# FluxML/Flux3D.jl

Hardware: AMD Instinct MI355X
Metric: chamfer_point_pairs_per_sec (higher is better)
Workload: dtype f32

## Files before the change

flux3d.jl_amd/csrc/chamfer.hip:

```cpp
#include <cmath>

#include "nn1_common.h"

using namespace fx3d;

#ifdef FX3D_PROBE
__device__ unsigned long long g_probe[4096 * 16];
#define FX3D_PROBE_MARK(k)                                                                   \
    do {                                                                                     \
        if (threadIdx.x == 0 && blockIdx.x < 4096) {                                         \
            g_probe[blockIdx.x * 16 + (k)] = __builtin_readcyclecounter();                   \
            if ((k) == 0) g_probe[blockIdx.x * 16 + 13] = wall_clock64();                    \
            if ((k) == 12) g_probe[blockIdx.x * 16 + 14] = wall_clock64();                   \
        }                                                                                    \
    } while (0)
__device__ unsigned long long g_probe2[256 * 16];
#define FX3D_PROBE_MARK2(k) do { if (threadIdx.x == 0 && blockIdx.x < 256) g_probe2[blockIdx.x * 16 + (k)] = __builtin_readcyclecounter(); } while (0)
__device__ unsigned long long g_probe3[16 * 16 * 8];
#define FX3D_PROBE_MARKW(k) do { if ((threadIdx.x & 63) == 0 && blockIdx.x < 16) g_probe3[(blockIdx.x * 16 + (threadIdx.x >> 6)) * 8 + (k)] = __builtin_readcyclecounter(); } while (0)
#else
#define FX3D_PROBE_MARK(k) do { } while (0)
#define FX3D_PROBE_MARK2(k) do { } while (0)
#define FX3D_PROBE_MARKW(k) do { } while (0)
#endif

namespace {

__device__ __forceinline__ void load4pts(const float *__restrict__ base, int p0, float (&px)[4],
                                         float (&py)[4], float (&pz)[4]) {
    const float4 *s4 = reinterpret_cast<const float4 *>(base + (size_t)p0 * 3);
    const float4 f0 = s4[0], f1 = s4[1], f2 = s4[2];
    px[0] = f0.x; py[0] = f0.y; pz[0] = f0.z;
    px[1] = f0.w; py[1] = f1.x; pz[1] = f1.y;
    px[2] = f1.z; py[2] = f1.w; pz[2] = f2.x;
    px[3] = f2.y; py[3] = f2.z; pz[3] = f2.w;
}

typedef _Float16 h8 __attribute__((ext_vector_type(8)));
typedef float f32x16 __attribute__((ext_vector_type(16)));
#ifndef FX3D_HFIFO
#define FX3D_HFIFO 5
#endif
constexpr int kHFifo = FX3D_HFIFO;
#ifndef FX3D_HRUNS_FROM
#define FX3D_HRUNS_FROM 16
#endif
constexpr int kHRunsFrom = FX3D_HRUNS_FROM;
constexpr int kScanU = 2;
#ifndef FX3D_HRUNCAP
#define FX3D_HRUNCAP 384
#endif
constexpr int kHRunCap = FX3D_HRUNCAP;
constexpr int kHItemCap = 64 * kHFifo > kHRunCap ? 64 * kHFifo : kHRunCap;
constexpr int kHFarCap = 64;
#ifndef FX3D_HBLKTRACK
#define FX3D_HBLKTRACK 1
#endif
constexpr bool kHBlkTrack = FX3D_HBLKTRACK != 0;
constexpr int kHIdBits = kHBlkTrack ? 7 : 6;
static_assert(kHChunkMax / (32 * kHLT) <= 64, "lane-tile ids live in the six (block ids: seven) low mantissa bits of the tracked keys");
constexpr float kKeyUp = kHBlkTrack ? 0x1.2p-16f : 0x1.2p-17f;
constexpr float kPadF16 = 65504.0f;
__device__ const unsigned short kHilbertCell[512] = {
    0, 1, 65, 64, 72, 73, 9, 8, 16, 24, 88, 80, 81, 89, 25, 17, 18, 26, 27, 19, 83, 91, 90, 82, 74, 10, 11, 75, 67, 3, 2, 66,
    130, 194, 195, 131, 139, 203, 202, 138, 146, 154, 155, 147, 211, 219, 218, 210, 209, 217, 153, 145, 144, 152, 216, 208, 200, 201, 137, 136, 128, 129, 193, 192,
    256, 257, 265, 264, 328, 329, 321, 320, 384, 448, 456, 392, 393, 457, 449, 385, 386, 450, 451, 387, 395, 459, 458, 394, 330, 322, 323, 331, 267, 259, 258, 266,
    274, 282, 283, 275, 339, 347, 346, 338, 402, 466, 467, 403, 411, 475, 474, 410, 409, 473, 465, 401, 400, 464, 472, 408, 344, 345, 337, 336, 272, 273, 281, 280,
    288, 296, 297, 289, 353, 361, 360, 352, 416, 480, 481, 417, 425, 489, 488, 424, 432, 496, 504, 440, 441, 505, 497, 433, 369, 368, 376, 377, 313, 312, 304, 305,
    306, 307, 315, 314, 378, 379, 371, 370, 434, 498, 506, 442, 443, 507, 499, 435, 427, 491, 490, 426, 418, 482, 483, 419, 355, 363, 362, 354, 290, 298, 299, 291,
    227, 235, 171, 163, 162, 170, 234, 226, 225, 224, 160, 161, 169, 168, 232, 233, 241, 240, 248, 249, 185, 184, 176, 177, 178, 242, 250, 186, 187, 251, 243, 179,
    115, 51, 59, 123, 122, 58, 50, 114, 113, 112, 120, 121, 57, 56, 48, 49, 41, 40, 104, 105, 97, 96, 32, 33, 34, 42, 106, 98, 99, 107, 43, 35,
    36, 44, 108, 100, 101, 109, 45, 37, 38, 39, 103, 102, 110, 111, 47, 46, 54, 55, 63, 62, 126, 127, 119, 118, 117, 53, 61, 125, 124, 60, 52, 116,
    180, 244, 252, 188, 189, 253, 245, 181, 182, 183, 191, 190, 254, 255, 247, 246, 238, 239, 175, 174, 166, 167, 231, 230, 229, 237, 173, 165, 164, 172, 236, 228,
    292, 300, 301, 293, 357, 365, 364, 356, 420, 484, 485, 421, 429, 493, 492, 428, 436, 500, 508, 444, 445, 509, 501, 437, 373, 372, 380, 381, 317, 316, 308, 309,
    310, 311, 319, 318, 382, 383, 375, 374, 438, 502, 510, 446, 447, 511, 503, 439, 431, 495, 494, 430, 422, 486, 487, 423, 359, 367, 366, 358, 294, 302, 303, 295,
    287, 286, 278, 279, 343, 342, 350, 351, 415, 479, 471, 407, 406, 470, 478, 414, 413, 477, 476, 412, 404, 468, 469, 405, 341, 349, 348, 340, 276, 284, 285, 277,
    269, 261, 260, 268, 332, 324, 325, 333, 397, 461, 460, 396, 388, 452, 453, 389, 390, 454, 462, 398, 399, 463, 455, 391, 327, 326, 334, 335, 271, 270, 262, 263,
    199, 198, 134, 135, 143, 142, 206, 207, 215, 223, 159, 151, 150, 158, 222, 214, 213, 221, 220, 212, 148, 156, 157, 149, 141, 205, 204, 140, 132, 196, 197, 133,
    69, 5, 4, 68, 76, 12, 13, 77, 85, 93, 92, 84, 20, 28, 29, 21, 22, 30, 94, 86, 87, 95, 31, 23, 15, 14, 78, 79, 71, 70, 6, 7,
};
constexpr size_t kHScratchBytes = (kHThreads / 64) * (32 * 8 + kHItemCap * 2 + 32 * 3 * 4) + 64 * 32;

__device__ __forceinline__ float vmin(float a, float b) {
    float r;
    asm("v_min_f32 %0, %1, %2" : "=v"(r) : "v"(a), "v"(b));
    return r;
}

__device__ __forceinline__ void split2h(float v, _Float16 &h, _Float16 &l) {
    h = (_Float16)v;
    l = (_Float16)(v - (float)h);
}

constexpr float kBetaC = 0x1.1p-18f;
constexpr float kBandB1 = 1.0f + 18.0f * kBetaC + 0x1p-20f;
constexpr float kBandA = 22.3f * kBetaC + 0x1p-19f;
__device__ __forceinline__ void make_pieces(float cx, float cy, float cz, h8 &p0, h8 &p1) {
    _Float16 hx, lx, hy, ly, hz, lz, n1, n2, n3;
    split2h(cx, hx, lx); split2h(cy, hy, ly); split2h(cz, hz, lz);
    const float n0 = ((cx * cx) + (cy * cy)) + (cz * cz);
    const float n = n0 + kBetaC * n0;
    n1 = (_Float16)n;
    const float r1 = n - (float)n1;
    n2 = (_Float16)r1;
    n3 = (_Float16)(r1 - (float)n2);
    const _Float16 z = (_Float16)0.0f;
    p0 = h8{hx, hx, lx, hy, hy, ly, hz, hz};
    p1 = h8{lz, n1, n2, n3, lx, ly, lz, z};
}

template <bool WANT_IDX, bool SPLITFUSE = false, bool PRUNE = false>
__global__ __launch_bounds__(kHThreads, 4) void nn1_f16_kernel(Nn1Params p) {
    extern __shared__ __attribute__((aligned(16))) float lds[];
    __shared__ __attribute__((aligned(16))) float red[4 * 4 * (kHThreads / 64) + 16];
    __shared__ int nfar[2];
    __shared__ unsigned short farlist[kHFarCap];
    constexpr int QB = (kHThreads / 64) * 32;

    const int L = blockIdx.x;
    const int per_cloud = p.tiles * p.nsplit;
    const bool by_xcd = 2 * p.B >= 8;
    const int slot = by_xcd ? L >> 3 : L;
    const int c = by_xcd ? (slot / per_cloud) * 8 + (L & 7) : slot / per_cloud;
    const int tile = (slot % per_cloud) / p.nsplit;
    const int split = (slot % per_cloud) % p.nsplit;
    if (c >= 2 * p.B) return;
    const int dir = c >= p.B ? 1 : 0;
    const int b = dir ? c - p.B : c;
    const int NQ = dir ? p.M : p.N;
    const int NC = dir ? p.N : p.M;
    if (tile >= (dir ? p.tiles_y : p.tiles_x)) return;
    if ((long long)split * p.chunk >= NC) return;
    const int ctail = (p.tail > 0 && p.nsplit == 1 && NC > p.chunk && NC - p.chunk <= p.tail) ? NC - p.chunk : 0;
    const int NCm = NC - ctail;
    const float *__restrict__ qb = (dir ? p.y : p.x) + (size_t)b * NQ * 3;
    const float *__restrict__ cb = (dir ? p.x : p.y) + (size_t)b * NC * 3;
    int32_t *idx_out = dir ? p.idx_y : p.idx_x;
    float *dmin_out = dir ? p.dmin_y : p.dmin_x;

    const int tid = threadIdx.x, lane = tid & 63;
    const int wv = __builtin_amdgcn_readfirstlane(tid >> 6);
    const int jq = lane & 31, hh = lane >> 5;
    const int CH = p.chunk;
    const int tpb = dir ? p.tpb_y : p.tpb;
    h8 *imgp = reinterpret_cast<h8 *>(lds);
    float4 *imgf = reinterpret_cast<float4 *>(lds);
    unsigned long long *wres = reinterpret_cast<unsigned long long *>(lds + 8 * (CH + 64));
    unsigned short *witems = reinterpret_cast<unsigned short *>(wres + (kHThreads / 64) * 32);
    float *wq = reinterpret_cast<float *>(witems + (kHThreads / 64) * kHItemCap);
    unsigned long long *qres = wres + wv * 32;
    unsigned short *items = witems + wv * kHItemCap;
    float *qtab = wq + wv * 96;
    const bool vec = (reinterpret_cast<uintptr_t>(cb) & 15) == 0;
    const bool one_shot = NCm <= CH;
    if (tid == 0) { nfar[0] = 0; nfar[1] = 0; }
    float qpre[3];
    {
        const int q0i = (tile * tpb) * QB + wv * 32 + jq;
        const int qc0 = q0i < NQ ? q0i : NQ - 1;
#pragma unroll
        for (int d = 0; d < 3; ++d) qpre[d] = qb[(size_t)qc0 * 3 + d];
    }
    if constexpr (PRUNE) {
        unsigned int *zc = reinterpret_cast<unsigned int *>(wres);
        for (int i = tid; i < 1040 + 16 * 256; i += kHThreads) zc[i] = 0u;
        int *gb = reinterpret_cast<int *>(wq + (kHThreads / 64) * 96) + 64 * 8;
        for (int i = tid; i < kHGroupsMax * 8; i += kHThreads) gb[i] = (i & 4) ? (int)0x80000000 : 0x7fffffff;
    }
    FX3D_PROBE_MARK(0);

    const bool own_chunk_only = p.nsplit > 1 && (long long)split * CH + (long long)p.nsplit * CH >= NCm;
    const int s_lo = own_chunk_only ? split * CH : 0;
    const int SN = own_chunk_only ? (NCm - s_lo < CH ? NCm - s_lo : CH) : NC;
    const float *__restrict__ sb = cb + (size_t)s_lo * 3;
    const bool parked = one_shot || own_chunk_only;
    float mu[3], cinf = 0.0f, varmax = 0.0f;
    float bxlo[3] = {0.f, 0.f, 0.f}, bxhi[3] = {0.f, 0.f, 0.f};
    bool allfin = true;
    {
        float mn[3] = {INFINITY, INFINITY, INFINITY}, mx[3] = {-INFINITY, -INFINITY, -INFINITY}, sm3[3] = {0.f, 0.f, 0.f};
        float sqt = 0.0f;
        const float pil[3] = {sb[0], sb[1], sb[2]};
        const int nsweep = (SN + kHThreads - 1) / kHThreads;
        for (int i0 = 0; i0 < nsweep; i0 += 4) {
            P3 v[4];
#pragma unroll
            for (int e = 0; e < 4; ++e) {
                const int pt = (i0 + e) * kHThreads + tid;
                v[e] = *reinterpret_cast<const P3 *>(sb + (size_t)(pt < SN ? pt : SN - 1) * 3);
            }
#pragma unroll
            for (int e = 0; e < 4; ++e) {
                const int pt = (i0 + e) * kHThreads + tid;
                mn[0] = fminf(mn[0], v[e].x); mx[0] = fmaxf(mx[0], v[e].x);
                mn[1] = fminf(mn[1], v[e].y); mx[1] = fmaxf(mx[1], v[e].y);
                mn[2] = fminf(mn[2], v[e].z); mx[2] = fmaxf(mx[2], v[e].z);
                if (pt < SN) {
                    sm3[0] = sm3[0] + v[e].x; sm3[1] = sm3[1] + v[e].y; sm3[2] = sm3[2] + v[e].z;
                    if (parked) imgf[((pt >> 5) * 2) * 32 + (pt & 31)] = float4{v[e].x, v[e].y, v[e].z, 0.0f};
                }
                if (((i0 + e) & 3) == (wv & 3) && pt < SN) {
                    sqt = __builtin_fmaf(v[e].x - pil[0], v[e].x - pil[0], sqt); sqt = __builtin_fmaf(v[e].y - pil[1], v[e].y - pil[1], sqt);
                    sqt = __builtin_fmaf(v[e].z - pil[2], v[e].z - pil[2], sqt);
                }
            }
        }
        FX3D_PROBE_MARK(5);
        {
            float4 lo4, hi4, st4;
            lo4.x = wave_min_l63(mn[0]); lo4.y = wave_min_l63(mn[1]); lo4.z = wave_min_l63(mn[2]); lo4.w = 0.0f;
            hi4.x = wave_max_l63(mx[0]); hi4.y = wave_max_l63(mx[1]); hi4.z = wave_max_l63(mx[2]); hi4.w = 0.0f;
            st4.x = wave_sum_l63(sm3[0]); st4.y = wave_sum_l63(sm3[1]); st4.z = wave_sum_l63(sm3[2]); st4.w = wave_sum_l63(sqt);
            if (lane == 63) {
                float4 *r4 = reinterpret_cast<float4 *>(red);
                r4[wv * 4] = lo4; r4[wv * 4 + 1] = hi4; r4[wv * 4 + 2] = st4;
            }
        }
        FX3D_PROBE_MARK(9);
        __syncthreads();
        FX3D_PROBE_MARK(10);
        static_assert(kHThreads / 64 == 16, "the cross-wave reduction below: one wave's row of 16 lanes, one lane per wave");
        if (wv == 0) {
            const float4 *r4 = reinterpret_cast<const float4 *>(red);
            const int w = lane & 15;
            float4 lo4 = r4[w * 4], hi4 = r4[w * 4 + 1], st4 = r4[w * 4 + 2];
#define NN1_ROW_MIN(v) v = fkey_inv(row_mm_key<false>(fkey(v)));
#define NN1_ROW_MAX(v) v = fkey_inv(row_mm_key<true>(fkey(v)));
#define NN1_ROW_SUM(v) v = v + dpp_mov<0xB1>(v); v = v + dpp_mov<0x4E>(v); v = v + dpp_mov<0x141>(v); v = v + dpp_mov<0x140>(v);
            NN1_ROW_MIN(lo4.x) NN1_ROW_MIN(lo4.y) NN1_ROW_MIN(lo4.z)
            NN1_ROW_MAX(hi4.x) NN1_ROW_MAX(hi4.y) NN1_ROW_MAX(hi4.z)
            NN1_ROW_SUM(st4.x) NN1_ROW_SUM(st4.y) NN1_ROW_SUM(st4.z) NN1_ROW_SUM(st4.w)
#undef NN1_ROW_MIN
#undef NN1_ROW_MAX
#undef NN1_ROW_SUM
            const float lo3[3] = {lo4.x, lo4.y, lo4.z}, hi3[3] = {hi4.x, hi4.y, hi4.z}, st3[3] = {st4.x, st4.y, st4.z};
            float m3[3], ci = 0.0f, vm = st4.w / fmaxf(0.25f * (float)SN, 1.0f);
            bool fin = true;
#pragma unroll
            for (int d = 0; d < 3; ++d) {
                const float lo = lo3[d], hi = hi3[d], st = st3[d];
                m3[d] = fminf(fmaxf(st / (float)SN, lo), hi);
                const float off = st / (float)SN - pil[d];
                vm = vm - off * off;
                ci = fmaxf(ci, fmaxf(hi - m3[d], m3[d] - lo));
                fin = fin && fabsf(st) < INFINITY;
            }
            if (lane == 0) {
                float4 *o4 = reinterpret_cast<float4 *>(red) + 4 * (kHThreads / 64);
                o4[0] = float4{m3[0], m3[1], m3[2], ci * 1.000001f};
                o4[1] = float4{vm, fin ? 1.0f : 0.0f, 0.0f, 0.0f};
                if (PRUNE) { o4[2] = float4{lo3[0], lo3[1], lo3[2], 0.0f}; o4[3] = float4{hi3[0], hi3[1], hi3[2], 0.0f}; }
            }
        }
        __syncthreads();
        {
            const float4 *o4 = reinterpret_cast<const float4 *>(red) + 4 * (kHThreads / 64);
            const float4 a = o4[0], b2 = o4[1];
            mu[0] = a.x; mu[1] = a.y; mu[2] = a.z; cinf = a.w;
            varmax = b2.x; allfin = b2.y != 0.0f;
            if (PRUNE) {
                const float4 l4 = o4[2], h4 = o4[3];
                bxlo[0] = l4.x; bxlo[1] = l4.y; bxlo[2] = l4.z; bxhi[0] = h4.x; bxhi[1] = h4.y; bxhi[2] = h4.z;
            }
        }
    }
    float rng = cinf;
    if (allfin && cinf < 1.0e16f && 3.0f * cinf * cinf > kRobustGate * varmax) {
        const float4 r = robust_range3<kHThreads, false>(sb, SN, parked, imgf, red, mu[0], mu[1], mu[2], cinf);
        mu[0] = r.x; mu[1] = r.y; mu[2] = r.z; rng = r.w;
    }
    const bool sane = allfin && cinf < 1.0e16f;
    float sc = 1.0f;
    if (sane && rng > 1.0e-30f) {
        int e;
        (void)frexpf(rng, &e);
        sc = ldexpf(1.0f, 7 - e);
    }
    auto uni = [](float v) { return __builtin_bit_cast(float, __builtin_amdgcn_readfirstlane(__builtin_bit_cast(int, v))); };
    mu[0] = uni(mu[0]); mu[1] = uni(mu[1]); mu[2] = uni(mu[2]); sc = uni(sc); rng = uni(rng); cinf = uni(cinf);
    const bool has_far = sane && rng < cinf;
    int fslot = 0;
    auto pieces = [&](float x, float y, float z, int pt, h8 &p0, h8 &p1) {
        const float sx = (x - mu[0]) * sc, sy = (y - mu[1]) * sc, sz = (z - mu[2]) * sc;
        if (!has_far) { make_pieces(sx, sy, sz, p0, p1); return; }
        const bool far = !(fmaxf(fmaxf(fabsf(sx), fabsf(sy)), fabsf(sz)) < 128.0f);
        make_pieces(far ? 0.f : sx, far ? 0.f : sy, far ? 0.f : sz, p0, p1);
        if (far) {
            p1[7] = (_Float16)kPadF16;
            const int f = atomicAdd(&nfar[fslot], 1);
            if (f < kHFarCap) farlist[f] = (unsigned short)pt;
        }
    };

    [[maybe_unused]] float4 *cs = nullptr, *qsw = nullptr;
    [[maybe_unused]] bool sorted_c = false;
    [[maybe_unused]] int qwlen = 0;
    [[maybe_unused]] float4 *boxes = nullptr;
    if constexpr (PRUNE) {
        cs = p.pscr + (size_t)blockIdx.x * p.pscr_stride;
        qsw = cs + kHChunkMax;
        boxes = reinterpret_cast<float4 *>(wq + (kHThreads / 64) * 96);
        unsigned int *ccnt = reinterpret_cast<unsigned int *>(wres);
        unsigned int *qtot = ccnt + 520;
        unsigned int *qwh = qtot + 520;
        const bool last_t = tile == (dir ? p.tiles_y : p.tiles_x) - 1;
        const int qw0 = tile * tpb * QB;
        const int qw1 = last_t || qw0 + tpb * QB > NQ ? NQ : qw0 + tpb * QB;
        qwlen = qw1 - qw0;
        const int cnt = NCm;
        const bool do_sort = sane && cnt >= 512;
        const bool sorted_q = do_sort && NQ <= 4 * kHThreads;
        P3 qv[4];
        if (sorted_q) {
#pragma unroll
            for (int e = 0; e < 4; ++e) {
                const int qp = 256 * wv + 64 * e + lane;
                qv[e] = *reinterpret_cast<const P3 *>(qb + (size_t)(qp < NQ ? qp : NQ - 1) * 3);
            }
        }
        FX3D_PROBE_MARK2(0);
        int *gbox = reinterpret_cast<int *>(boxes + 64 * 2);
        auto group_box = [&](int wrow, float x, float y, float z) {
            int *g = gbox + (wrow >> 5) * 8;
            atomicMin(g + 0, fkey((x - mu[0]) * sc)); atomicMin(g + 1, fkey((y - mu[1]) * sc)); atomicMin(g + 2, fkey((z - mu[2]) * sc));
            atomicMax(g + 4, fkey((x - mu[0]) * sc)); atomicMax(g + 5, fkey((y - mu[1]) * sc)); atomicMax(g + 6, fkey((z - mu[2]) * sc));
        };
        if (do_sort) {
            float4 cv[4];
#pragma unroll
            for (int e = 0; e < 4; ++e) {
                const int pt = e * kHThreads + tid;
                cv[e] = float4{0.f, 0.f, 0.f, 0.f};
                if (pt < cnt) cv[e] = imgf[((pt >> 5) * 2) * 32 + (pt & 31)];
            }
            FX3D_PROBE_MARK2(1);
            float inv[3], off[3], cfl[3], cfh[3];
#pragma unroll
            for (int d = 0; d < 3; ++d) {
                const float fr = has_far ? 0.125f * rng : 128.0f / sc;
                const float flo = fmaxf(bxlo[d], mu[d] - fr), fhi = fminf(bxhi[d], mu[d] + fr);
                inv[d] = fhi > flo ? 8.0f / (fhi - flo) : 0.0f;
                off[d] = -flo * inv[d];
                cfl[d] = flo; cfh[d] = fhi;
            }
            auto cell = [&](float x, float y, float z) -> unsigned int {
                const unsigned int ux = (unsigned int)(int)fminf(fmaxf(__builtin_fmaf(x, inv[0], off[0]), 0.0f), 7.0f);
                const unsigned int uy = (unsigned int)(int)fminf(fmaxf(__builtin_fmaf(y, inv[1], off[1]), 0.0f), 7.0f);
                const unsigned int uz = (unsigned int)(int)fminf(fmaxf(__builtin_fmaf(z, inv[2], off[2]), 0.0f), 7.0f);
                return ux | (uy << 3) | (uz << 6);
            };

            unsigned int ccr[4], qcr[4];
            auto count_cells = [&](bool valid, unsigned int t, auto &&add) -> unsigned int {
                unsigned int rank = 0u;
                bool mine = valid;
                const unsigned int tn = (unsigned int)__builtin_amdgcn_update_dpp((int)~t, (int)t, 0x111, 0xF, 0xF, false);
                if (__builtin_popcountll(__ballot(valid && t == tn)) >= 8) {
                    unsigned long long rem = __ballot(valid);
                    for (int it = 0; it < 12 && rem; ++it) {
                        const unsigned int t0 = (unsigned int)__builtin_amdgcn_readlane((int)t, __builtin_ctzll(rem));
                        const unsigned long long grp = __ballot(mine && t == t0);
                        rem &= ~grp;
                        if (__builtin_popcountll(grp) < 4) continue;
                        unsigned int base = 0u;
                        if ((int)lane == __builtin_ctzll(grp)) base = add(t0, (unsigned int)__builtin_popcountll(grp));
                        base = (unsigned int)__builtin_amdgcn_readlane((int)base, __builtin_ctzll(grp));
                        if (mine && t == t0) {
                            rank = base + __builtin_amdgcn_mbcnt_hi((unsigned int)(grp >> 32), __builtin_amdgcn_mbcnt_lo((unsigned int)grp, 0u));
                            mine = false;
                        }
                    }
                }
                if (mine) rank = add(t, 1u);
                return rank;
            };
#pragma unroll
            for (int e = 0; e < 4; ++e) {
                const int pt = e * kHThreads + tid;
                const unsigned int t = pt < cnt ? cell(cv[e].x, cv[e].y, cv[e].z) : 0u;
                ccr[e] = (t << 16) | count_cells(pt < cnt, t, [&](unsigned int c, unsigned int n) { return atomicAdd(&ccnt[c], n); });
            }
            int *qbb = reinterpret_cast<int *>(boxes + 64 * 2 + kHGroupsMax * 2 - 2);
            if (sorted_q) {
                int kl[3] = {0x7fffffff, 0x7fffffff, 0x7fffffff}, kh[3] = {(int)0x80000000, (int)0x80000000, (int)0x80000000};
#pragma unroll
                for (int e = 0; e < 4; ++e) {
                    const int qp = 256 * wv + 64 * e + lane;
                    if (qp < NQ) {
                        const int k3[3] = {fkey(qv[e].x), fkey(qv[e].y), fkey(qv[e].z)};
#pragma unroll
                        for (int d = 0; d < 3; ++d) { kl[d] = kl[d] < k3[d] ? kl[d] : k3[d]; kh[d] = kh[d] > k3[d] ? kh[d] : k3[d]; }
                    }
                }
#pragma unroll
                for (int d = 0; d < 3; ++d) {
                    int a = row_mm_key<false>(kl[d]), b2 = row_mm_key<true>(kh[d]);
                    a = imm<false>(a, dpp_keepi<0x142, 0xA>(a)); a = imm<false>(a, dpp_keepi<0x143, 0xC>(a));
                    b2 = imm<true>(b2, dpp_keepi<0x142, 0xA>(b2)); b2 = imm<true>(b2, dpp_keepi<0x143, 0xC>(b2));
                    if (lane == 63) { atomicMin(qbb + d, a); atomicMax(qbb + 4 + d, b2); }
                }
            }
            FX3D_PROBE_MARK2(2);
            __syncthreads();
            FX3D_PROBE_MARK2(3);
            float qinv[3] = {0.f, 0.f, 0.f}, qoff[3] = {0.f, 0.f, 0.f};
            if (sorted_q) {
                const float ext = fmaxf(fmaxf(cfh[0] - cfl[0], cfh[1] - cfl[1]), cfh[2] - cfl[2]);
#pragma unroll
                for (int d = 0; d < 3; ++d) {
                    const float ql = fkey_inv(qbb[d]), qh = fkey_inv(qbb[4 + d]);
                    const float grow = qh - ql > 4.0f * ext ? 0.25f * ext : ext;
                    const float lo = fmaxf(ql, cfl[d] - grow), hi = fminf(qh, cfh[d] + grow);
                    qinv[d] = hi > lo && hi - lo < INFINITY ? 8.0f / (hi - lo) : 0.0f;
                    qoff[d] = qinv[d] != 0.0f ? -lo * qinv[d] : 0.0f;
                }
            }
            auto qcell = [&](float x, float y, float z) -> unsigned int {
                const unsigned int ux = (unsigned int)(int)fminf(fmaxf(__builtin_fmaf(x, qinv[0], qoff[0]), 0.0f), 7.0f);
                const unsigned int uy = (unsigned int)(int)fminf(fmaxf(__builtin_fmaf(y, qinv[1], qoff[1]), 0.0f), 7.0f);
                const unsigned int uz = (unsigned int)(int)fminf(fmaxf(__builtin_fmaf(z, qinv[2], qoff[2]), 0.0f), 7.0f);
                return ux | (uy << 3) | (uz << 6);
            };
            auto curve_scan = [&](unsigned int *a) {
                unsigned int tc[8];
                {
                    const uint4 h = *reinterpret_cast<const uint4 *>(kHilbertCell + 8 * lane);
                    tc[0] = h.x & 0xffffu; tc[1] = h.x >> 16; tc[2] = h.y & 0xffffu; tc[3] = h.y >> 16;
                    tc[4] = h.z & 0xffffu; tc[5] = h.z >> 16; tc[6] = h.w & 0xffffu; tc[7] = h.w >> 16;
                }
                unsigned int c8[8], tot = 0u;
#pragma unroll
                for (int k = 0; k < 8; ++k) { c8[k] = a[tc[k]]; tot += c8[k]; }
                unsigned int inc = tot;
#pragma unroll
                for (int o = 1; o < 64; o <<= 1) {
                    const unsigned int v = __shfl_up(inc, o, 64);
                    if (lane >= o) inc += v;
                }
                unsigned int run = inc - tot;
#pragma unroll
                for (int k = 0; k < 8; ++k) { a[tc[k]] = run; run += c8[k]; }
            };
            if (wv == 0) curve_scan(ccnt);
            if (sorted_q) {
#pragma unroll
                for (int e = 0; e < 4; ++e) {
                    const int qp = 256 * wv + 64 * e + lane;
                    const unsigned int t = qp < NQ ? qcell(qv[e].x, qv[e].y, qv[e].z) : 0u;
                    qcr[e] = (t << 16) | count_cells(qp < NQ, t, [&](unsigned int c, unsigned int n) {
                                 const unsigned int sh = 16u * (c & 1u);
                                 const unsigned int old = atomicAdd(&qwh[wv * 256 + (c >> 1)], n << sh);
                                 atomicAdd(&qtot[c], n);
                                 return (old >> sh) & 0xffffu;
                             });
                }
            }
            FX3D_PROBE_MARK2(4);
            __syncthreads();
            FX3D_PROBE_MARK2(5);
#pragma unroll
            for (int e = 0; e < 4; ++e) {
                const int pt = e * kHThreads + tid;
                if (pt < cnt) {
                    const int pos = (int)(ccnt[ccr[e] >> 16] + (ccr[e] & 0xffffu));
                    imgf[((pos >> 5) * 2) * 32 + (pos & 31)] = float4{cv[e].x, cv[e].y, cv[e].z, __builtin_bit_cast(float, pt)};
                }
            }
            sorted_c = true;
            if (sorted_q) {
                if (wv == 1) {
                    curve_scan(qtot);
                } else if (wv >= 2 && wv < 6) {
                    const int w2 = tid - 128;
                    unsigned int run = 0u;
#pragma unroll
                    for (int w = 0; w < 16; ++w) {
                        const unsigned int v = qwh[w * 256 + w2];
                        qwh[w * 256 + w2] = run;
                        run += v;
                    }
                }
            }
            FX3D_PROBE_MARK2(6);
            __syncthreads();
            FX3D_PROBE_MARK2(7);
            if (sorted_q) {
#pragma unroll
                for (int e = 0; e < 4; ++e) {
                    const int qp = 256 * wv + 64 * e + lane;
                    if (qp < NQ) {
                        const unsigned int t = qcr[e] >> 16;
                        const int rank = (int)(qtot[t] + ((qwh[wv * 256 + (t >> 1)] >> (16u * (t & 1u))) & 0xffffu) + (qcr[e] & 0xffffu));
                        if (rank >= qw0 && rank < qw1) {
                            qsw[rank - qw0] = float4{qv[e].x, qv[e].y, qv[e].z, __builtin_bit_cast(float, qp)};
                            group_box(rank - qw0, qv[e].x, qv[e].y, qv[e].z);
                        }
                    }
                }
            }
        }
        if (!sorted_q) {
            for (int q0 = qw0 + wv * 64; q0 < qw1; q0 += kHThreads) {
                const int qp = q0 + lane;
                const P3 r = *reinterpret_cast<const P3 *>(qb + (size_t)(qp < qw1 ? qp : qw1 - 1) * 3);
                if (qp < qw1) qsw[qp - qw0] = float4{r.x, r.y, r.z, __builtin_bit_cast(float, qp)};
                const int kx = fkey((r.x - mu[0]) * sc), ky = fkey((r.y - mu[1]) * sc), kz = fkey((r.z - mu[2]) * sc);
                const int lx = row_mm_key<false>(kx), ly = row_mm_key<false>(ky), lz = row_mm_key<false>(kz);
                const int hx = row_mm_key<true>(kx), hy = row_mm_key<true>(ky), hz = row_mm_key<true>(kz);
                if ((lane & 15) == 0 && qp < qw1) {
                    int *g = gbox + ((qp - qw0) >> 5) * 8;
                    atomicMin(g + 0, lx); atomicMin(g + 1, ly); atomicMin(g + 2, lz);
                    atomicMax(g + 4, hx); atomicMax(g + 5, hy); atomicMax(g + 6, hz);
                }
            }
        }
        FX3D_PROBE_MARK2(8);
    }
    FX3D_PROBE_MARK(1);

    const float cm2 = 3.0f * (fminf(cinf * sc, 128.0f) * fminf(cinf * sc, 128.0f));
    float qr[3], da = 0.0f;
    float da_far = 0.0f;
    [[maybe_unused]] float dpr = INFINITY;
    bool qfin = true;
    int qi = 0;
    bool qok = true;
    h8 bq;
    double acc = 0.0;

    const int jfirst = split * CH, jstep = p.nsplit * CH;
    for (int j0 = jfirst; j0 < NCm; j0 += jstep) {
        const int cnt = (NCm - j0) < CH ? (NCm - j0) : CH;
        const int cnt_pad = (cnt + 32 * kHLT - 1) / (32 * kHLT) * (32 * kHLT);
        if (j0 > jfirst) __syncthreads();
        if constexpr (PRUNE) {
            for (int tl = tid >> 4; tl * 64 < cnt_pad + 64; tl += kHThreads / 16) {
                float4 r4[4];
#pragma unroll
                for (int k = 0; k < 4; ++k) {
                    const int pt = tl * 64 + k * 16 + (tid & 15);
                    r4[k] = float4{0.f, 0.f, 0.f, 0.f};
                    if (pt < cnt) r4[k] = imgf[((pt >> 5) * 2) * 32 + (pt & 31)];
                }
                float lo3[3] = {INFINITY, INFINITY, INFINITY}, hi3[3] = {-INFINITY, -INFINITY, -INFINITY};
#pragma unroll
                for (int k = 0; k < 4; ++k) {
                    const int pt = tl * 64 + k * 16 + (tid & 15), i0 = ((pt >> 5) * 2) * 32 + (pt & 31);
                    h8 p0, p1;
                    if (pt < cnt) {
                        pieces(r4[k].x, r4[k].y, r4[k].z, pt, p0, p1);
                        const int id = sorted_c ? __builtin_bit_cast(int, r4[k].w) : j0 + pt;
                        cs[pt] = float4{r4[k].x, r4[k].y, r4[k].z, __builtin_bit_cast(float, id)};
                        const float b3[3] = {(r4[k].x - mu[0]) * sc, (r4[k].y - mu[1]) * sc, (r4[k].z - mu[2]) * sc};
#pragma unroll
                        for (int d = 0; d < 3; ++d) { lo3[d] = vmin(lo3[d], b3[d]); hi3[d] = -vmin(-hi3[d], -b3[d]); }
                    } else {
                        make_pieces(0.f, 0.f, 0.f, p0, p1);
                        p1[7] = (_Float16)kPadF16;
                    }
                    imgp[i0] = p0;
                    imgp[i0 + 32] = p1;
                }
                float bl[3], bh[3];
#pragma unroll
                for (int d = 0; d < 3; ++d) { bl[d] = fkey_inv(row_mm_key<false>(fkey(lo3[d]))); bh[d] = fkey_inv(row_mm_key<true>(fkey(hi3[d]))); }
                if ((tid & 15) == 0 && tl < 64) {
                    boxes[tl * 2] = float4{bl[0], bl[1], bl[2], 0.0f};
                    boxes[tl * 2 + 1] = float4{bh[0], bh[1], bh[2], 0.0f};
                }
            }
        } else
        for (int pt = tid; pt < cnt_pad + 64; pt += kHThreads) {
            const int i0 = ((pt >> 5) * 2) * 32 + (pt & 31);
            h8 p0, p1;
            if (pt < cnt) {
                if (parked) {
                    const float4 r = imgf[i0];
                    pieces(r.x, r.y, r.z, pt, p0, p1);
                } else {
                    const P3 r = *reinterpret_cast<const P3 *>(cb + (size_t)(j0 + pt) * 3);
                    pieces(r.x, r.y, r.z, pt, p0, p1);
                }
            } else {
                make_pieces(0.f, 0.f, 0.f, p0, p1);
                p1[7] = (_Float16)kPadF16;
            }
            imgp[i0] = p0;
            imgp[i0 + 32] = p1;
        }
        __syncthreads();
        FX3D_PROBE_MARK(j0 == jfirst ? 2 : 6);
        FX3D_PROBE_MARKW(0);

        const int nf = nfar[fslot];
        if (tid == 0) nfar[fslot ^ 1] = 0;
        fslot ^= 1;
        const bool far_ok = nf <= kHFarCap;
        const bool last_tile = tile == (dir ? p.tiles_y : p.tiles_x) - 1;
        for (int tp = 0; tp < tpb || (last_tile && one_shot); ++tp) {
            if ((tile * tpb + tp) * QB >= NQ) break;
            if constexpr (PRUNE) {
                if (tp * QB + wv * 32 >= qwlen) continue;
            }
            if (j0 == jfirst) {
                qi = (tile * tpb + tp) * QB + wv * 32 + jq;
                if constexpr (PRUNE) {
                    const int wpos = tp * QB + wv * 32 + jq;
                    const float4 q4 = qsw[wpos < qwlen ? wpos : qwlen - 1];
                    qr[0] = q4.x; qr[1] = q4.y; qr[2] = q4.z;
                    qi = wpos < qwlen ? __builtin_bit_cast(int, q4.w) : NQ;
                } else if (tp == 0) {
#pragma unroll
                    for (int d = 0; d < 3; ++d) qr[d] = qpre[d];
                } else {
                    const int qc1 = qi < NQ ? qi : NQ - 1;
#pragma unroll
                    for (int d = 0; d < 3; ++d) qr[d] = qb[(size_t)qc1 * 3 + d];
                }
                float m0 = -2.0f * ((qr[0] - mu[0]) * sc), m1 = -2.0f * ((qr[1] - mu[1]) * sc), m2 = -2.0f * ((qr[2] - mu[2]) * sc);
                float S = (fabsf(m0) + fabsf(m1)) + fabsf(m2);
                float sq = 1.0f, fl_s = 0.0f;
                if (S >= 3.0e4f && S < 0x1p28f) {
                    int e;
                    (void)frexpf(S, &e);
                    sq = ldexpf(1.0f, 14 - e);
                    m0 *= sq; m1 *= sq; m2 *= sq; S *= sq;
                    fl_s = 0x1p-15f;
                }
                qok = S < 3.0e4f;
                qfin = fabsf(qr[0]) + fabsf(qr[1]) + fabsf(qr[2]) < INFINITY;
                const float qn = 0.25f * ((m0 * m0 + m1 * m1) + m2 * m2) / sq;
                da = kBandA * qn + 0x1p-24f * (S + 4.0f) + fl_s;
                {
                    const float c2 = sq * cm2;
                    da_far = 2.1f * kBetaC * c2 + 2.0f * kBetaC * sqrtf(qn * c2) + 0x1p-19f * qn + 0x1p-24f * (S + 4.0f) + fl_s;
                }
                if constexpr (PRUNE) {
                    dpr = qok && sq == 1.0f ? qn + 2.0f * kBetaC * (cm2 + qn) + 0x1p-23f * (S + 4.0f) : INFINITY;
                }
                _Float16 hx, lx, hy, ly, hz, lz;
                split2h(qok ? m0 : 0.f, hx, lx); split2h(qok ? m1 : 0.f, hy, ly); split2h(qok ? m2 : 0.f, hz, lz);
                const _Float16 one = (_Float16)sq, pad = (_Float16)kPadF16;
                bq = hh == 0 ? h8{hx, lx, hx, hy, ly, hy, hz, lz} : h8{hz, one, one, one, lx, ly, lz, pad};
                if (hh == 0) {
                    qres[jq] = ~0ull;
                    qtab[jq * 3 + 0] = qr[0]; qtab[jq * 3 + 1] = qr[1]; qtab[jq * 3 + 2] = qr[2];
                }
            }

            float tm = INFINITY, fk[kHFifo];
#pragma unroll
            for (int s = 0; s < kHFifo; ++s) fk[s] = INFINITY;
            const unsigned int keymask = ~((1u << kHIdBits) - 1u);

            static_assert(kHLT == 2, "the rotation below is written for lane tiles of two blocks");
            const int nblk = cnt_pad / 32;
            f32x16 zero;
#pragma unroll
            for (int r = 0; r < 16; ++r) zero[r] = 0.0f;
#define NN1_FOLD(ACC, FIRST)                                                                                         \
            {                                                                                                        \
                const float t0 = min3f(ACC[0], ACC[1], ACC[2]), t1 = min3f(ACC[3], ACC[4], ACC[5]);                  \
                const float t2 = min3f(ACC[6], ACC[7], ACC[8]), t3 = min3f(ACC[9], ACC[10], ACC[11]);                \
                const float t4 = min3f(ACC[12], ACC[13], ACC[14]);                                                   \
                const float t5 = min3f(t0, t1, t2), t6 = min3f(t3, t4, ACC[15]);                                     \
                tm = (FIRST) ? vmin(t5, t6) : min3f(tm, t5, t6);       \
            }
#define NN1_TRACK_ID(LT)                                                                                             \
            {                                                                                                        \
                float key;                                                                                           \
                asm("v_and_or_b32 %0, %1, %2, %3" : "=v"(key) : "v"(tm), "v"(keymask), "s"(LT));                     \
                _Pragma("unroll") for (int s_ = kHFifo - 1; s_ > 0; --s_) fk[s_] = __builtin_amdgcn_fmed3f(fk[s_ - 1], fk[s_], key);    \
                fk[0] = vmin(fk[0], key);                                                                            \
            }
#define NN1_TRACK() { NN1_TRACK_ID(lt) ++lt; }
#define NN1_CLOSE(ACC, ODD, LT)                                                                                      \
            if constexpr (kHBlkTrack) { NN1_FOLD(ACC, true) NN1_TRACK_ID(2 * (LT) + (ODD)) }                           \
            else { NN1_FOLD(ACC, !(ODD)) if (ODD) NN1_TRACK_ID(LT) }
#define NN1_STEP(ISSUE, FOLD, ODD, OFF)                                                                              \
            __builtin_amdgcn_s_setprio(0);                                                                           \
            ISSUE = __builtin_amdgcn_mfma_f32_32x32x16_f16(an, bq, zero, 0, 0, 0);                                   \
            an = pa[(OFF) * 64];                                                                                     \
            __builtin_amdgcn_s_setprio(1);                                                                           \
            NN1_CLOSE(FOLD, ODD, lt)                                                                                 \
            if (ODD) ++lt;
            if constexpr (!PRUNE) {
            const h8 *pa = imgp + hh * 32 + jq;
            f32x16 acc0, acc1, acc2;
            h8 an = pa[0];
            acc0 = __builtin_amdgcn_mfma_f32_32x32x16_f16(an, bq, zero, 0, 0, 0); an = pa[1 * 64];
            acc1 = __builtin_amdgcn_mfma_f32_32x32x16_f16(an, bq, zero, 0, 0, 0); an = pa[2 * 64];
            pa += 3 * 64;
            int lt = 0;
            int nb = 2;
            for (; nb + 6 <= nblk; nb += 6) {
                NN1_STEP(acc2, acc0, 0, 0) NN1_STEP(acc0, acc1, 1, 1) NN1_STEP(acc1, acc2, 0, 2)
                NN1_STEP(acc2, acc0, 1, 3) NN1_STEP(acc0, acc1, 0, 4) NN1_STEP(acc1, acc2, 1, 5)
                pa += 6 * 64;
            }
            if (nblk - nb == 4) {
                NN1_STEP(acc2, acc0, 0, 0) NN1_STEP(acc0, acc1, 1, 1) NN1_STEP(acc1, acc2, 0, 2) NN1_STEP(acc2, acc0, 1, 3)
                NN1_CLOSE(acc1, 0, lt) NN1_CLOSE(acc2, 1, lt)
            } else if (nblk - nb == 2) {
                NN1_STEP(acc2, acc0, 0, 0) NN1_STEP(acc0, acc1, 1, 1)
                NN1_CLOSE(acc2, 0, lt) NN1_CLOSE(acc0, 1, lt)
            } else {
                NN1_CLOSE(acc0, 0, lt) NN1_CLOSE(acc1, 1, lt)
            }
            } else {
            const int nltp = nblk / kHLT;
            float bd = INFINITY;
            {
                const int4 *gq = reinterpret_cast<const int4 *>(boxes + 64 * 2) + (tp * (kHThreads / 64) + wv) * 2;
                const int4 gl = gq[0], gh = gq[1];
                const float qlx = fkey_inv(gl.x), qly = fkey_inv(gl.y), qlz = fkey_inv(gl.z);
                const float qhx = fkey_inv(gh.x), qhy = fkey_inv(gh.y), qhz = fkey_inv(gh.z);
                if (lane < nltp) {
                    const float4 lo = boxes[lane * 2], hi = boxes[lane * 2 + 1];
                    const float gx = fmaxf(fmaxf(lo.x - qhx, qlx - hi.x), 0.0f), gy = fmaxf(fmaxf(lo.y - qhy, qly - hi.y), 0.0f);
                    const float gz = fmaxf(fmaxf(lo.z - qhz, qlz - hi.z), 0.0f);
                    bd = (gx * gx + gy * gy) + gz * gz;
                }
            }
            const unsigned long long all_lt = nltp >= 64 ? ~0ull : (1ull << nltp) - 1ull;
            unsigned long long todo = all_lt, done = 0ull;
            if (sorted_c) {
                todo = __ballot(bd == 0.0f);
                if (!todo) {
                    const float bmin = wave_min_f(bd);
                    todo = bmin < INFINITY ? __ballot(bd == bmin) : all_lt;
                }
            }
            const h8 *pbase = imgp + hh * 32 + jq;
            for (int phase = 0; phase < 2; ++phase) {
                if (phase == 1) {
                    if (done == all_lt) break;
                    const float kb = fk[0];
                    const float bb = __builtin_fmaf(fabsf(kb), kKeyUp, kb);
                    const float dj = fminf(bb, __shfl_xor(bb, 32, 64)) + dpr;
                    const float ucut = wave_max_f(__builtin_fmaf(dj, 1.0f + 0x1p-9f, 0x1p-8f));
                    const bool keep = !(bd > ucut) || !(dj == dj);
                    todo = (__ballot(!(dj == dj)) ? all_lt : __ballot(keep)) & all_lt & ~done;
                    if (!todo) break;
                }
                done |= todo;
                unsigned long long mk = todo;
                int nrem = __builtin_popcountll(mk) - 1;
#define NN1_NEXT(T) { T = nltp; if (mk) { T = __builtin_ctzll(mk); mk &= mk - 1ull; } }
                int ta, tb;
                NN1_NEXT(ta) NN1_NEXT(tb)
                f32x16 acc0, acc1, acc2;
                const h8 *pn = pbase + ta * (kHLT * 64);
                h8 an = pn[0];
                acc0 = __builtin_amdgcn_mfma_f32_32x32x16_f16(an, bq, zero, 0, 0, 0); an = pn[64];
                pn = pbase + tb * (kHLT * 64);
                acc1 = __builtin_amdgcn_mfma_f32_32x32x16_f16(an, bq, zero, 0, 0, 0); an = pn[0];
#define NN1_PSTEP(ISSUE, FOLD, ODD, LT, NEXT)                                                                         \
                __builtin_amdgcn_s_setprio(0);                                                                       \
                ISSUE = __builtin_amdgcn_mfma_f32_32x32x16_f16(an, bq, zero, 0, 0, 0);                               \
                an = NEXT;                                                                                           \
                __builtin_amdgcn_s_setprio(1);                                                                       \
                NN1_CLOSE(FOLD, ODD, LT)
                while (nrem >= 3) {
                    int tc, td, te;
                    NN1_NEXT(tc) NN1_NEXT(td) NN1_NEXT(te)
                    nrem -= 3;
                    const h8 *pc = pbase + tc * (kHLT * 64), *pd = pbase + td * (kHLT * 64);
                    NN1_PSTEP(acc2, acc0, 0, ta, pn[64])
                    NN1_PSTEP(acc0, acc1, 1, ta, pc[0])
                    pn = pbase + te * (kHLT * 64);
                    NN1_PSTEP(acc1, acc2, 0, tb, pc[64])
                    NN1_PSTEP(acc2, acc0, 1, tb, pd[0])
                    NN1_PSTEP(acc0, acc1, 0, tc, pd[64])
                    NN1_PSTEP(acc1, acc2, 1, tc, pn[0])
                    ta = td; tb = te;
                }
                if (nrem == 2) {
                    int tc;
                    NN1_NEXT(tc)
                    const h8 *pc = pbase + tc * (kHLT * 64);
                    NN1_PSTEP(acc2, acc0, 0, ta, pn[64])
                    NN1_PSTEP(acc0, acc1, 1, ta, pc[0])
                    NN1_PSTEP(acc1, acc2, 0, tb, pc[64])
                    NN1_PSTEP(acc2, acc0, 1, tb, pc[64])
                    NN1_CLOSE(acc1, 0, tc) NN1_CLOSE(acc2, 1, tc)
                } else if (nrem == 1) {
                    NN1_PSTEP(acc2, acc0, 0, ta, pn[64])
                    NN1_PSTEP(acc0, acc1, 1, ta, pn[64])
                    NN1_CLOSE(acc2, 0, tb) NN1_CLOSE(acc0, 1, tb)
                } else {
                    NN1_CLOSE(acc0, 0, ta) NN1_CLOSE(acc1, 1, ta)
                }
#undef NN1_PSTEP
#undef NN1_NEXT
                __builtin_amdgcn_s_setprio(0);
#ifdef FX3D_PROBE_COUNT
                if ((threadIdx.x & 63) == 0) atomicAdd(&g_probe[4095 * 16 + 6 + phase], (unsigned long long)__builtin_popcountll(todo));
#endif
            }
            }
#undef NN1_STEP
#undef NN1_CLOSE
#undef NN1_TRACK
#undef NN1_TRACK_ID
#undef NN1_FOLD
            __builtin_amdgcn_s_setprio(0);
            float ft[kHFifo];
#pragma unroll
            for (int s = 0; s < kHFifo; ++s) ft[s] = fk[s];
            const float ka = fk[0];
            const float best = __builtin_fmaf(fabsf(ka), kKeyUp, ka);
            FX3D_PROBE_MARK(tp == 0 ? 3 : 7);
            FX3D_PROBE_MARKW(tp == 0 ? 1 : 3);

            {
                int opq;
                asm volatile("s_mov_b32 %0, 0" : "=s"(opq));
                const int lane = (int)(threadIdx.x & 63) + opq, jq = lane & 31, hh = lane >> 5;
                const float m = fminf(best, __shfl_xor(best, 32, 64));
                const float thr1 = fminf(__builtin_fmaf(m, kBandB1, da), __builtin_fmaf(m, 1.0f + 0x1p-20f, da_far));
                const float thr1k = __builtin_fmaf(fabsf(thr1), kKeyUp, thr1);
                const bool usable = sane && far_ok && qok && m < INFINITY;
                const bool slow = !usable || !(fk[kHFifo - 1] > thr1k);
                const unsigned long long sb = __ballot(slow);
                unsigned int qslow = (unsigned int)sb | (unsigned int)(sb >> 32);
                const bool retry = __builtin_popcount(qslow) > 2;
                bool fifo_done = false;
                const bool nonfinite = !sane || __ballot(!qfin) != 0;
                const int nlt = nblk / kHLT;
                int lt2 = 0;
                const bool runs = retry && __builtin_popcount(qslow) >= kHRunsFrom;
#ifdef FX3D_PROBE_COUNT
                if ((threadIdx.x & 63) == 0) {
                    unsigned long long *pc = &g_probe[4095 * 16];
                    atomicAdd(&pc[0], 1ull); atomicAdd(&pc[1], qslow ? 1ull : 0ull); atomicAdd(&pc[2], retry ? 1ull : 0ull);
                    atomicAdd(&pc[3], runs ? 1ull : 0ull); atomicAdd(&pc[4], (unsigned long long)__builtin_popcount(qslow));
                    atomicAdd(&pc[5], (unsigned long long)__builtin_popcountll(__ballot(!usable)));
                }
#endif
                const int lt2_end = runs ? nblk : nlt;
                do {
                    int nitems = 0;
                    if (!retry && fifo_done) {
                        const int qsl = __builtin_ctz(qslow);
                        qslow &= qslow - 1;
                        const float qq[3] = {qtab[qsl * 3], qtab[qsl * 3 + 1], qtab[qsl * 3 + 2]};
                        unsigned long long kbest = ~0ull;
                        for (int h = 0; h < 2; ++h) {
                            if (!((sb >> (32 * h + qsl)) & 1ull)) continue;
                            for (int r0 = 4 * (2 * lane + h); r0 < cnt; r0 += kScanU * 512) {
                                float cx[kScanU][4], cy[kScanU][4], cz[kScanU][4];
                                [[maybe_unused]] int cid[kScanU][4];
#pragma unroll
                                for (int u = 0; u < kScanU; ++u) {
                                    const int jl0 = r0 + 512 * u;
                                    if constexpr (PRUNE) {
#pragma unroll
                                        for (int r = 0; r < 4; ++r) {
                                            const float4 v = cs[jl0 + r < cnt ? jl0 + r : cnt - 1];
                                            cx[u][r] = v.x; cy[u][r] = v.y; cz[u][r] = v.z; cid[u][r] = __builtin_bit_cast(int, v.w);
                                        }
                                    } else if (vec && jl0 + 4 <= cnt) {
                                        load4pts(cb, j0 + jl0, cx[u], cy[u], cz[u]);
                                    } else {
#pragma unroll
                                        for (int r = 0; r < 4; ++r) {
                                            const int jc = jl0 + r < cnt ? jl0 + r : cnt - 1;
                                            const float *src = cb + (size_t)(j0 + jc) * 3;
                                            cx[u][r] = src[0]; cy[u][r] = src[1]; cz[u][r] = src[2];
// ... 382 lines not shown
```

Measured before the change: 14560 billion.

## Compute query group boxes in-wave with DPP instead of LDS atomics

Drops the shared-memory atomicMin/atomicMax accumulation of per-32-query bounding boxes during query staging. Each wave now derives its query box directly from its own query coordinates with row min/max keys, a DPP combine and readlanes. The cloud points loaded for the stats pass are kept in registers, so the parked float4 image is written only when the robust-range path needs it. The sort reads those registers instead of reloading from LDS, and pad-tile init moves to a dedicated thread group. This trades LDS atomics, extra LDS stores and a zero-init loop for more register pressure and subtle dependence on the key-sign trick via xor with -hh.

```diff
diff --git a/flux3d.jl_amd/csrc/chamfer.hip b/flux3d.jl_amd/csrc/chamfer.hip
--- a/flux3d.jl_amd/csrc/chamfer.hip
+++ b/flux3d.jl_amd/csrc/chamfer.hip
@@ -164,8 +164,8 @@
     if constexpr (PRUNE) {
         unsigned int *zc = reinterpret_cast<unsigned int *>(wres);
         for (int i = tid; i < 1040 + 16 * 256; i += kHThreads) zc[i] = 0u;
-        int *gb = reinterpret_cast<int *>(wq + (kHThreads / 64) * 96) + 64 * 8;
-        for (int i = tid; i < kHGroupsMax * 8; i += kHThreads) gb[i] = (i & 4) ? (int)0x80000000 : 0x7fffffff;
+        int *qb0 = reinterpret_cast<int *>(wq + (kHThreads / 64) * 96) + 64 * 8 + (kHGroupsMax - 1) * 8;
+        if (tid < 8) qb0[tid] = (tid & 4) ? (int)0x80000000 : 0x7fffffff;
     }
     FX3D_PROBE_MARK(0);
 
@@ -177,6 +177,7 @@
     float mu[3], cinf = 0.0f, varmax = 0.0f;
     float bxlo[3] = {0.f, 0.f, 0.f}, bxhi[3] = {0.f, 0.f, 0.f};
     bool allfin = true;
+    [[maybe_unused]] P3 vk[4];
     {
         float mn[3] = {INFINITY, INFINITY, INFINITY}, mx[3] = {-INFINITY, -INFINITY, -INFINITY}, sm3[3] = {0.f, 0.f, 0.f};
         float sqt = 0.0f;
@@ -197,12 +198,13 @@
                 mn[2] = fminf(mn[2], v[e].z); mx[2] = fmaxf(mx[2], v[e].z);
                 if (pt < SN) {
                     sm3[0] = sm3[0] + v[e].x; sm3[1] = sm3[1] + v[e].y; sm3[2] = sm3[2] + v[e].z;
-                    if (parked) imgf[((pt >> 5) * 2) * 32 + (pt & 31)] = float4{v[e].x, v[e].y, v[e].z, 0.0f};
+                    if (parked && !PRUNE) imgf[((pt >> 5) * 2) * 32 + (pt & 31)] = float4{v[e].x, v[e].y, v[e].z, 0.0f};
                 }
                 if (((i0 + e) & 3) == (wv & 3) && pt < SN) {
                     sqt = __builtin_fmaf(v[e].x - pil[0], v[e].x - pil[0], sqt); sqt = __builtin_fmaf(v[e].y - pil[1], v[e].y - pil[1], sqt);
                     sqt = __builtin_fmaf(v[e].z - pil[2], v[e].z - pil[2], sqt);
                 }
+                if constexpr (PRUNE) vk[e] = v[e];
             }
         }
         FX3D_PROBE_MARK(5);
@@ -265,6 +267,18 @@
         }
     }
     float rng = cinf;
+    if constexpr (PRUNE) {
+        static_assert(kHChunkMax <= 4 * kHThreads, "the cloud pass of a pruned launch is one iteration of four sweeps");
+        const bool sane0 = allfin && cinf < 1.0e16f;
+        if (!(sane0 && NCm >= 512) || 3.0f * cinf * cinf > kRobustGate * varmax) {
+#pragma unroll
+            for (int e = 0; e < 4; ++e) {
+                const int pt = e * kHThreads + tid;
+                if (pt < SN) imgf[((pt >> 5) * 2) * 32 + (pt & 31)] = float4{vk[e].x, vk[e].y, vk[e].z, 0.0f};
+            }
+            __syncthreads();
+        }
+    }
     if (allfin && cinf < 1.0e16f && 3.0f * cinf * cinf > kRobustGate * varmax) {
         const float4 r = robust_range3<kHThreads, false>(sb, SN, parked, imgf, red, mu[0], mu[1], mu[2], cinf);
         mu[0] = r.x; mu[1] = r.y; mu[2] = r.z; rng = r.w;
@@ -319,20 +333,8 @@
             }
         }
         FX3D_PROBE_MARK2(0);
-        int *gbox = reinterpret_cast<int *>(boxes + 64 * 2);
-        auto group_box = [&](int wrow, float x, float y, float z) {
-            int *g = gbox + (wrow >> 5) * 8;
-            atomicMin(g + 0, fkey((x - mu[0]) * sc)); atomicMin(g + 1, fkey((y - mu[1]) * sc)); atomicMin(g + 2, fkey((z - mu[2]) * sc));
-            atomicMax(g + 4, fkey((x - mu[0]) * sc)); atomicMax(g + 5, fkey((y - mu[1]) * sc)); atomicMax(g + 6, fkey((z - mu[2]) * sc));
-        };
         if (do_sort) {
-            float4 cv[4];
-#pragma unroll
-            for (int e = 0; e < 4; ++e) {
-                const int pt = e * kHThreads + tid;
-                cv[e] = float4{0.f, 0.f, 0.f, 0.f};
-                if (pt < cnt) cv[e] = imgf[((pt >> 5) * 2) * 32 + (pt & 31)];
-            }
+            const P3(&cv)[4] = vk;
             FX3D_PROBE_MARK2(1);
             float inv[3], off[3], cfl[3], cfh[3];
 #pragma unroll
@@ -491,27 +493,15 @@
                     if (qp < NQ) {
                         const unsigned int t = qcr[e] >> 16;
                         const int rank = (int)(qtot[t] + ((qwh[wv * 256 + (t >> 1)] >> (16u * (t & 1u))) & 0xffffu) + (qcr[e] & 0xffffu));
-                        if (rank >= qw0 && rank < qw1) {
-                            qsw[rank - qw0] = float4{qv[e].x, qv[e].y, qv[e].z, __builtin_bit_cast(float, qp)};
-                            group_box(rank - qw0, qv[e].x, qv[e].y, qv[e].z);
-                        }
+                        if (rank >= qw0 && rank < qw1) qsw[rank - qw0] = float4{qv[e].x, qv[e].y, qv[e].z, __builtin_bit_cast(float, qp)};
                     }
                 }
             }
         }
         if (!sorted_q) {
-            for (int q0 = qw0 + wv * 64; q0 < qw1; q0 += kHThreads) {
-                const int qp = q0 + lane;
-                const P3 r = *reinterpret_cast<const P3 *>(qb + (size_t)(qp < qw1 ? qp : qw1 - 1) * 3);
-                if (qp < qw1) qsw[qp - qw0] = float4{r.x, r.y, r.z, __builtin_bit_cast(float, qp)};
-                const int kx = fkey((r.x - mu[0]) * sc), ky = fkey((r.y - mu[1]) * sc), kz = fkey((r.z - mu[2]) * sc);
-                const int lx = row_mm_key<false>(kx), ly = row_mm_key<false>(ky), lz = row_mm_key<false>(kz);
-                const int hx = row_mm_key<true>(kx), hy = row_mm_key<true>(ky), hz = row_mm_key<true>(kz);
-                if ((lane & 15) == 0 && qp < qw1) {
-                    int *g = gbox + ((qp - qw0) >> 5) * 8;
-                    atomicMin(g + 0, lx); atomicMin(g + 1, ly); atomicMin(g + 2, lz);
-                    atomicMax(g + 4, hx); atomicMax(g + 5, hy); atomicMax(g + 6, hz);
-                }
+            for (int qp = qw0 + tid; qp < qw1; qp += kHThreads) {
+                const P3 r = *reinterpret_cast<const P3 *>(qb + (size_t)qp * 3);
+                qsw[qp - qw0] = float4{r.x, r.y, r.z, __builtin_bit_cast(float, qp)};
             }
         }
         FX3D_PROBE_MARK2(8);
@@ -534,7 +524,14 @@
         const int cnt_pad = (cnt + 32 * kHLT - 1) / (32 * kHLT) * (32 * kHLT);
         if (j0 > jfirst) __syncthreads();
         if constexpr (PRUNE) {
-            for (int tl = tid >> 4; tl * 64 < cnt_pad + 64; tl += kHThreads / 16) {
+            if (tid >= kHThreads - 128) {
+                const int u = tid - (kHThreads - 128);
+                h8 p0, p1;
+                make_pieces(0.f, 0.f, 0.f, p0, p1);
+                p1[7] = (_Float16)kPadF16;
+                imgp[cnt_pad * 2 + u] = (u & 32) ? p1 : p0;
+            }
+            for (int tl = tid >> 4; tl * 64 < cnt_pad; tl += kHThreads / 16) {
                 float4 r4[4];
 #pragma unroll
                 for (int k = 0; k < 4; ++k) {
@@ -542,7 +539,7 @@
                     r4[k] = float4{0.f, 0.f, 0.f, 0.f};
                     if (pt < cnt) r4[k] = imgf[((pt >> 5) * 2) * 32 + (pt & 31)];
                 }
-                float lo3[3] = {INFINITY, INFINITY, INFINITY}, hi3[3] = {-INFINITY, -INFINITY, -INFINITY};
+                float lo3[3] = {INFINITY, INFINITY, INFINITY}, nhi3[3] = {INFINITY, INFINITY, INFINITY};
 #pragma unroll
                 for (int k = 0; k < 4; ++k) {
                     const int pt = tl * 64 + k * 16 + (tid & 15), i0 = ((pt >> 5) * 2) * 32 + (pt & 31);
@@ -553,7 +550,7 @@
                         cs[pt] = float4{r4[k].x, r4[k].y, r4[k].z, __builtin_bit_cast(float, id)};
                         const float b3[3] = {(r4[k].x - mu[0]) * sc, (r4[k].y - mu[1]) * sc, (r4[k].z - mu[2]) * sc};
 #pragma unroll
-                        for (int d = 0; d < 3; ++d) { lo3[d] = vmin(lo3[d], b3[d]); hi3[d] = -vmin(-hi3[d], -b3[d]); }
+                        for (int d = 0; d < 3; ++d) { lo3[d] = vmin(lo3[d], b3[d]); nhi3[d] = vmin(nhi3[d], -b3[d]); }
                     } else {
                         make_pieces(0.f, 0.f, 0.f, p0, p1);
                         p1[7] = (_Float16)kPadF16;
@@ -563,8 +560,8 @@
                 }
                 float bl[3], bh[3];
 #pragma unroll
-                for (int d = 0; d < 3; ++d) { bl[d] = fkey_inv(row_mm_key<false>(fkey(lo3[d]))); bh[d] = fkey_inv(row_mm_key<true>(fkey(hi3[d]))); }
-                if ((tid & 15) == 0 && tl < 64) {
+                for (int d = 0; d < 3; ++d) { bl[d] = fkey_inv(row_mm_key<false>(fkey(lo3[d]))); bh[d] = fkey_inv(row_mm_key<true>(fkey(-nhi3[d]))); }
+                if ((tid & 15) == 0) {
                     boxes[tl * 2] = float4{bl[0], bl[1], bl[2], 0.0f};
                     boxes[tl * 2 + 1] = float4{bh[0], bh[1], bh[2], 0.0f};
                 }
@@ -711,10 +708,16 @@
             const int nltp = nblk / kHLT;
             float bd = INFINITY;
             {
-                const int4 *gq = reinterpret_cast<const int4 *>(boxes + 64 * 2) + (tp * (kHThreads / 64) + wv) * 2;
-                const int4 gl = gq[0], gh = gq[1];
-                const float qlx = fkey_inv(gl.x), qly = fkey_inv(gl.y), qlz = fkey_inv(gl.z);
-                const float qhx = fkey_inv(gh.x), qhy = fkey_inv(gh.y), qhz = fkey_inv(gh.z);
+                int gk[3];
+#pragma unroll
+                for (int d = 0; d < 3; ++d) {
+                    int k = fkey((qr[d] - mu[d]) * sc) ^ -hh;
+                    k = row_mm_key<false>(k);
+                    gk[d] = imm<false>(k, dpp_keepi<0x142, 0xA>(k));
+                }
+                const float qlx = fkey_inv(__builtin_amdgcn_readlane(gk[0], 31)), qhx = fkey_inv(~__builtin_amdgcn_readlane(gk[0], 63));
+                const float qly = fkey_inv(__builtin_amdgcn_readlane(gk[1], 31)), qhy = fkey_inv(~__builtin_amdgcn_readlane(gk[1], 63));
+                const float qlz = fkey_inv(__builtin_amdgcn_readlane(gk[2], 31)), qhz = fkey_inv(~__builtin_amdgcn_readlane(gk[2], 63));
                 if (lane < nltp) {
                     const float4 lo = boxes[lane * 2], hi = boxes[lane * 2 + 1];
                     const float gx = fmaxf(fmaxf(lo.x - qhx, qlx - hi.x), 0.0f), gy = fmaxf(fmaxf(lo.y - qhy, qly - hi.y), 0.0f);
```

New measurement: 14870 billion, median of 5. +2.1%, better.
